# IntelLabs/bayesian-torch

Hardware: AMD Instinct MI355X
Metric: MC-samples/sec (Bayesian-ResNet18, 224^2, bs=64) (higher is better)
Workload: dtype bf16

## Files before the change

### bayesian_torch_amd/csrc/btx_contract.h

```cpp
#pragma once
#include <hip/hip_runtime.h>
#include <stdint.h>
#include "btx_rng.h"
#include "btx_plan.h"

typedef __attribute__((ext_vector_type(8))) __bf16 bf16x8;
typedef __attribute__((ext_vector_type(4))) __bf16 bf16x4;
typedef __attribute__((ext_vector_type(4))) float f32x4;
typedef __attribute__((ext_vector_type(8))) float f32x8;
typedef __attribute__((ext_vector_type(16))) float f32x16;
typedef __attribute__((ext_vector_type(4))) uint32_t u32x4;
typedef __attribute__((ext_vector_type(2))) uint32_t u32x2;

namespace btx {

constexpr int NTHREADS = 512;
constexpr int ACTS_OFF = 0;
constexpr int SIGN_OFF = NG * BM * 16;
constexpr int WMU_OFF = SIGN_OFF + NG * BM * 4;
constexpr int WDL_OFF = WMU_OFF + NG * BN * 16;
constexpr int STAGE_BYTES = WDL_OFF + NG * BN * 16;
constexpr int LDS_BYTES = 2 * STAGE_BYTES;

struct FastDiv {
  uint32_t m, sh;
};
static inline FastDiv make_fastdiv(uint32_t d) {
  FastDiv f;
  uint32_t l = 0;
  while ((1ull << l) < d) ++l;
  f.m = (uint32_t)((((1ull << l) - d) << 32) / d + 1);
  f.sh = (l < 1 ? l : 1) | ((l > 0 ? l - 1 : 0) << 8);
  return f;
}
__device__ __forceinline__ uint32_t fdiv(uint32_t x, const FastDiv& f) {
  const uint32_t t = __umulhi(x, f.m);
  return (t + ((x - t) >> (f.sh & 31u))) >> (f.sh >> 8);
}
static inline void sign_keys(const BtxRng* rng, uint32_t stream, uint32_t* ka, uint32_t* kb) {
  const BtxPhilox4 k = btx_philox4x32_10(0u, rng->sample_idx, rng->layer_id, stream, (uint32_t)rng->seed,
                                         (uint32_t)(rng->seed >> 32));
  *ka = k.x[0];
  *kb = k.x[1];
}
__device__ __forceinline__ void fdivmod(uint32_t x, const FastDiv& f, uint32_t d, uint32_t& q, uint32_t& r) {
  q = fdiv(x, f);
  r = x - q * d;
}

struct ContractParams {
  const void* x;
  const float* mu;
  const float* rho;
  const float* mu_b;
  const float* rho_b;
  void* out;
  float* partial;
  const float* eps_w;
  const float* eps_b;
  const int8_t* sign_in;
  const int8_t* sign_out;
  int NB, D, H, W, C, Cg;
  int Do, Ho, Wo, N, Ng;
  int KD, KH, KW;
  int sd, sh, sw, pd, ph, pw, dd, dh, dw;
  int M, K;
  int mtiles, ntiles, groups, ksplits, kper;
  int transposed;
  int pointwise;
  uint32_t seed_lo, seed_hi, sample, layer;
  const uint32_t* sample_ptr;
  uint32_t kin_a, kin_b, kout_a, kout_b;
  const float* ep_scale;
  const float* ep_shift;
  const void* ep_res;
  int ep_relu;
  int out_bf16;
  int sign_unaligned;
  uint32_t x_bytes, w_bytes;
  int pt_G, pt_R, pt_Rp, pt_Wp, pt_PP, pt_NI, pt_rtiles;
  FastDiv fd_Wo, fd_Ho, fd_Do, fd_ptWp, fd_ptRp, fd_ptR;
  FastDiv fd_inner, fd_ksplits, fd_ntiles, fd_Cg, fd_KW, fd_KH, fd_rtiles;
  FastDiv fd_mtiles;
  int swap_signs;
  int par_major, par_Mq, par_Mqp, par_Hh, par_Wh;
  FastDiv fd_par_Mqp, fd_par_Hh, fd_par_Wh;
  FastDiv fd_sd, fd_sh, fd_sw;
  int wg_order;
  int pt_nw, pt_astage, pt_lds;
  int pt_kg;
  int pt_lds_g;
  int pt_taps;
  int pt_wide;
  int sp_Hq, sp_Wq;
  int st_sbytes;
  void* wt;
  uint32_t wt_bytes, wt_delta_off;
  int wt_ready;
  int pt_tall, pt_P, pt_Wt, pt_ncs;
  FastDiv fd_P, fd_Wt, fd_ncs;
  int lanes, lane_nwg;
// ... 708 lines not shown
```

### bayesian_torch_amd/csrc/btx_contract_taps.h

```cpp
#pragma once
#include <type_traits>
#include "btx_contract.h"
#include "btx_contract_dma.h"
#include "btx_epilogue.h"
#include "btx_mma.h"

namespace btx {

__device__ __forceinline__ void dma16s(__amdgpu_buffer_rsrc_t rsrc, uint32_t voff, uint32_t soff,
                                       unsigned char* lds_wave_base) {
  __builtin_amdgcn_raw_ptr_buffer_load_lds(rsrc, (__attribute__((address_space(3))) void*)lds_wave_base, 16, voff, soff,
                                           0, 0);
}

template <int N>
__device__ __forceinline__ void end_stage() {
  asm volatile("s_waitcnt vmcnt(%0)\n\ts_waitcnt lgkmcnt(0)\n\ts_barrier" ::"n"(N) : "memory");
}

template <int I, int N, class F>
__device__ __forceinline__ void static_for(F&& f) {
  if constexpr (I < N) {
    f(std::integral_constant<int, I>{});
    static_for<I + 1, N>(f);
// ... 5 lines not shown
template <int T>
constexpr int tp_pieces(int t) {
  constexpr int PST = T - 3;
  constexpr int PPS = (TP_MAXNI + PST - 1) / PST;
  if (t < 0) t += T;
  if (t >= PST) return 0;
  int n = 0;
  for (int i = 0; i < PPS; ++i)
    if (t + PST * i < TP_MAXNI) ++n;
  return n;
}

template <int PREC, int KIND, int KH, int KW, int KG, bool WIDE = false>
__global__ __launch_bounds__(256 * KG, 2) void contract_taps_kernel(const ContractParams) {
  static_assert(!WIDE || (PREC == 1 && KG == 1 && KIND == 0), "wide tile: bf16 Reparameterization, one K-group");
  constexpr int K2 = (KIND == 1 || WIDE) ? 1 : 0;
  BTX_SECTION_PARAMS(p, logical);
  constexpr int NW = 4, NT = 256, MI = 2, T = KH * KW;
  static_assert(T >= 5 && T <= 32, "tap-unrolled kernel: 5..32 taps");
  constexpr int MAXNI = TP_MAXNI;
  constexpr int PST = T - 3;
  constexpr int WOPS = K2 ? 2 : 1;
  using ACT = typename std::conditional<PREC == 1, __bf16, float>::type;
  constexpr int G = (PREC == 1) ? 8 : 4;
  constexpr int BK = NG * G;
  constexpr int ESZ = (int)sizeof(ACT);
  extern __shared__ __attribute__((aligned(16))) unsigned char smem_all[];

  uint32_t smp = p.sample;
  if (p.sample_ptr) smp = sample_word_scalar(p.sample_ptr);

  const int tid = threadIdx.x & 255;
  const int lane = tid & 63;
  const int l31 = lane & 31;
  const int h = lane >> 5;
  const int wave_all = __builtin_amdgcn_readfirstlane((int)(threadIdx.x >> 6));
  const int wave = wave_all & 3;
  const int kg = (KG == 1) ? 0 : (wave_all >> 2);
  unsigned char* const smem = smem_all + kg * p.pt_lds_g;

  uint32_t u_mtile, u_rem, u_split, u_ntile, u_group, u_t;
  const uint32_t ntg = (uint32_t)(WIDE ? p.ntiles >> 1 : p.ntiles);
  if (p.wg_order) fdivmod((uint32_t)logical, p.fd_mtiles, (uint32_t)p.mtiles, u_rem, u_mtile);
  else fdivmod((uint32_t)logical, p.fd_inner, ntg * (uint32_t)(p.groups * p.ksplits), u_mtile, u_rem);
  fdivmod(u_rem, p.fd_ksplits, (uint32_t)p.ksplits, u_t, u_split);
  fdivmod(u_t, p.fd_ntiles, ntg, u_group, u_ntile);
  const int mtile = (int)u_mtile, split = (int)u_split, ntile = (int)u_ntile, group = (int)u_group;

  const bool tall = p.pt_tall != 0;
  uint32_t u_ig, u_rt;
  if (tall) fdivmod((uint32_t)mtile, p.fd_ncs, (uint32_t)p.pt_ncs, u_rt, u_ig);
  else fdivmod((uint32_t)mtile, p.fd_rtiles, (uint32_t)p.pt_rtiles, u_ig, u_rt);
  const int img0 = tall ? 0 : (int)u_ig * p.pt_G, row0 = (int)u_rt * p.pt_R, col0 = tall ? (int)u_ig * p.pt_Wt : 0;
  auto patch_src = [&](int q, bool& ok) __attribute__((always_inline)) -> uint32_t {
    uint32_t ut, upc, ugi, upr;
    fdivmod((uint32_t)q, p.fd_ptWp, (uint32_t)p.pt_Wp, ut, upc);
    int img, ih, iw;
    if (tall) {
      fdivmod((uint32_t)row0 + ut, p.fd_P, (uint32_t)p.pt_P, ugi, upr);
      img = (int)ugi; ih = (int)upr - p.ph; iw = col0 + (int)upc - p.pw;
      ok = (int)ut < p.pt_Rp;
    } else {
      fdivmod(ut, p.fd_ptRp, (uint32_t)p.pt_Rp, ugi, upr);
      img = img0 + (int)ugi; ih = row0 + (int)upr - p.ph; iw = (int)upc - p.pw;
      ok = true;
    }
    ok = ok && img < p.NB && (unsigned)ih < (unsigned)p.H && (unsigned)iw < (unsigned)p.W;
    return (uint32_t)((img * p.H + ih) * p.W + iw);
  };
  const int ncb_total = p.Cg / BK;
  const int cb_per = p.kper / BK;
  const int cb0 = split * cb_per + kg * (cb_per / KG);
  const int ncb = (KG == 1) ? min(ncb_total, cb0 + cb_per) - cb0 : cb_per / KG;
  const int a_stage = p.pt_astage, s_stage = p.pt_astage >> 4;
  const int PT_A_OFF = 0, PT_S_OFF = 2 * a_stage, PT_W_OFF = 2 * a_stage + 2 * s_stage;
  const int PT_X_OFF = PT_W_OFF + PT_WD * DW_STAGE;

  const __amdgpu_buffer_rsrc_t x_rsrc = __builtin_amdgcn_make_buffer_rsrc((void*)p.x, 0, p.x_bytes, 0x00020000);
  const __amdgpu_buffer_rsrc_t wt_rsrc = __builtin_amdgcn_make_buffer_rsrc((void*)p.wt, 0, p.wt_bytes, 0x00020000);

  const uint32_t w_voff = (uint32_t)lane * 16u + (uint32_t)wave * 1024u;
  const uint32_t w_sbase = (uint32_t)(group * p.ntiles + (WIDE ? 2 * ntile : ntile)) * (uint32_t)(p.K / G) * 1024u;
  const uint32_t w_second = WIDE ? (uint32_t)(p.K / G) * 1024u : p.wt_delta_off;
  const uint32_t CgG = (uint32_t)(p.Cg / G);
  const int w_lds = PT_W_OFF + wave * 1024;
  int wslot = 0;
  auto issue_w = [&](uint32_t tap, uint32_t cb, int slot) __attribute__((always_inline)) {
    const uint32_t soff = w_sbase + (tap * CgG + cb * (uint32_t)NG) * 1024u;
    unsigned char* ld = smem + w_lds + slot * DW_STAGE;
    dma16s(wt_rsrc, w_voff, soff, ld);
    if constexpr (K2) dma16s(wt_rsrc, w_voff, soff + w_second, ld + 4096);
  };
  if (ncb > 0) issue_w(0u, (uint32_t)cb0, 0);

  uint32_t sg_off[2];
  bool sg_ok[2];
  uint32_t* const pix_tab = (uint32_t*)(smem + PT_S_OFF + s_stage);
#pragma unroll
  for (int j = 0; j < 2; ++j) {
    const int q = tid + NT * j;
    sg_ok[j] = q < p.pt_PP;
    bool inside;
    const uint32_t ipix = patch_src(sg_ok[j] ? q : 0, inside);
    sg_off[j] = ipix * (uint32_t)p.C + (uint32_t)(group * p.Cg);
    if (q * 4 < s_stage) pix_tab[q] = (sg_ok[j] && inside) ? sg_off[j] : 0xffffffffu;
    if (p.sign_in)
      sg_ok[j] = sg_ok[j] && inside;
  }
  asm volatile("s_waitcnt lgkmcnt(0)\n\ts_barrier" ::: "memory");

  const int g_lane = (lane & 3) ^ ((lane >> 4) & 3);
  uint32_t pp_boff[MAXNI];
  uint32_t pmask = 0;
  uint32_t pp_e[MAXNI];
#pragma unroll
// ... 6 lines not shown
    const int q = 16 * (wave + NW * j) + (lane >> 2);
    uint32_t bo = DMA_OOB;
    if (j < p.pt_NI && q < p.pt_PP) {
      const uint32_t e = pp_e[j];
      if (e != 0xffffffffu) bo = (e + (uint32_t)(G * g_lane)) * (uint32_t)ESZ;
    }
    pp_boff[j] = bo;
    if (j < p.pt_NI && 16 * (wave + NW * j) < p.pt_PP) {
      pmask |= 1u << j;
      if (ncb > 0)
        dma16(x_rsrc, bo == DMA_OOB ? DMA_OOB : bo + (uint32_t)(cb0 * BK * ESZ), smem + PT_A_OFF + (wave + NW * j) * 1024);
    }
  }
  pmask = __builtin_amdgcn_readfirstlane(pmask);
  if (ncb > 0) {
    issue_w(1u, (uint32_t)cb0, 1);
    issue_w(2u, (uint32_t)cb0, 2);
  }

  RngLive rl = {smp, p.kin_a, p.kin_b, p.kout_a, p.kout_b};
  if (p.sample_ptr || p.lanes > 1) {
    rl.sample = __builtin_amdgcn_readfirstlane(smp);
    if constexpr (KIND == 1) {
      const uint32_t si = p.swap_signs ? 3u : 2u, so = p.swap_signs ? 2u : 3u;
      const BtxPhilox4 ki = btx_philox4x32_10(0u, rl.sample, p.layer, si, p.seed_lo, p.seed_hi);
      const BtxPhilox4 ko = btx_philox4x32_10(0u, rl.sample, p.layer, so, p.seed_lo, p.seed_hi);
      rl.kin_a = __builtin_amdgcn_readfirstlane(ki.x[0]); rl.kin_b = __builtin_amdgcn_readfirstlane(ki.x[1]);
      rl.kout_a = __builtin_amdgcn_readfirstlane(ko.x[0]); rl.kout_b = __builtin_amdgcn_readfirstlane(ko.x[1]);
    }
  }

  auto write_signs = [&](int slot, int cb) __attribute__((always_inline)) {
    if constexpr (KIND == 1) {
      unsigned char* ss = smem + PT_S_OFF + slot * s_stage;
#pragma unroll
      for (int j = 0; j < 2; ++j) {
        if (sg_ok[j]) {
          const uint32_t off = sg_off[j] + (uint32_t)(cb * BK);
          uint32_t w;
          if (p.sign_in) w = sign_word_explicit(p.sign_in, off, p.x_bytes / (uint32_t)ESZ);
          else w = btx_sign_word(off >> 5, rl.kin_a, rl.kin_b);
          if constexpr (G == 4) w <<= 8 * ((off >> 4) & 1);
          *(uint32_t*)(ss + (tid + NT * j) * 4) = w;
        }
      }
    }
  };

  int q0[MI];
#pragma unroll
  for (int mi = 0; mi < MI; ++mi) {
    const int pl = wave * 64 + mi * 32 + l31;
    uint32_t ut, uc, ugi, ur;
    if (tall) {
      fdivmod((uint32_t)pl, p.fd_Wt, (uint32_t)p.pt_Wt, ur, uc);
      q0[mi] = ((int)ur < p.pt_R) ? (int)ur * p.pt_Wp + (int)uc : 0;
    } else {
      fdivmod((uint32_t)pl, p.fd_Wo, (uint32_t)p.Wo, ut, uc);
      fdivmod(ut, p.fd_ptR, (uint32_t)p.pt_R, ugi, ur);
      const int c = (int)uc, r = (int)ur, gi = (int)ugi;
      const bool ok = (gi < p.pt_G) && (img0 + gi < p.NB) && (row0 + r < p.Ho);
      q0[mi] = ok ? (gi * p.pt_Rp + r) * p.pt_Wp + c : 0;
    }
  }
  const int row_step = p.dh * p.pt_Wp;

  constexpr bool ZI = (PREC == 1 && KG == 1);
  f32x16 accm[MI][2], accd[MI][2];
  auto clear_acc = [&](int a0) __attribute__((always_inline)) {
#pragma unroll
    for (int a = 0; a < MI; ++a)
#pragma unroll
      for (int b = 0; b < 2; ++b)
#pragma unroll
        for (int r = 0; r < 16; ++r)
          if (a >= a0) { accm[a][b][r] = 0.f; accd[a][b][r] = 0.f; }
  };
  if (!ZI || ncb <= 0) clear_acc(0);

  using Frag = StageFragT<MI>;
  auto load_frag = [&](Frag& f, int aslot, int toffv, int wsl, auto mia_tag) __attribute__((always_inline)) {
    constexpr int MIA = decltype(mia_tag)::value;
    const unsigned char* as = smem + PT_A_OFF + aslot * a_stage;
    const unsigned char* ss = smem + PT_S_OFF + aslot * s_stage;
    const unsigned char* ws = smem + PT_W_OFF + wsl * DW_STAGE;
    int q[MI];
#pragma unroll
    for (int mi = 0; mi < MI; ++mi) q[mi] = q0[mi] + toffv;
#pragma unroll
    for (int kk = 0; kk < NG / 2; ++kk) {
      const int row = 2 * kk + h;
#pragma unroll
      for (int mi = 0; mi < MIA; ++mi) f.a[kk][mi] = *(const u32x4*)(as + q[mi] * 64 + ((row ^ ((q[mi] >> 2) & 3)) * 16));
#pragma unroll
      for (int ni = 0; ni < 2; ++ni) f.wm[kk][ni] = *(const u32x4*)(ws + (row * BN + ni * 32 + l31) * 16);
    }
    if constexpr (KIND == 1) {
#pragma unroll
      for (int mi = 0; mi < MIA; ++mi) f.sw[mi] = *(const uint32_t*)(ss + q[mi] * 4);
    }
  };

  if (ncb > 0) {
    write_signs(0, cb0);
    asm volatile("s_waitcnt vmcnt(%0)\n\ts_waitcnt lgkmcnt(0)\n\ts_barrier" ::"n"(KG == 1 ? WOPS : 2 * WOPS) : "memory");
    Frag fa, fb;
    const int nvalid_px = tall ? p.pt_R * p.pt_Wt : min(p.pt_G, p.NB - img0) * min(p.pt_R, p.Ho - row0) * p.Wo;
    const bool mi1_dead = wave * 64 + 32 >= nvalid_px;
    auto kloop = [&](auto mia_tag) __attribute__((always_inline)) {
    constexpr int MIA = decltype(mia_tag)::value;
    if constexpr (KG == 1) load_frag(fa, 0, 0, 0, mia_tag);
    auto block = [&](auto par_tag, auto first_tag, int cbi, bool last) __attribute__((always_inline)) {
      constexpr int PAR = decltype(par_tag)::value;
      constexpr bool FIRST = decltype(first_tag)::value;
      static_for<0, T>([&](auto t_tag) __attribute__((always_inline)) {
        constexpr int t = decltype(t_tag)::value;
        constexpr int sp = (PAR * T + t) & 1;
        Frag& cur = (KG == 1 && sp) ? fb : fa;
        Frag& nxt = (KG == 1 && sp) ? fa : fb;
        asm volatile("" : "+v"(q0[0]), "+v"(q0[1]));
        constexpr int t3 = (t + 3) % T, c3 = (t + 3) / T;
        if constexpr (c3 == 0) {
          issue_w((uint32_t)t3, (uint32_t)(cb0 + cbi), (wslot + 3) & 3);
        } else {
          if (!last) issue_w((uint32_t)t3, (uint32_t)(cb0 + cbi + 1), (wslot + 3) & 3);
        }
        constexpr int KP = tp_pieces<T>(t);
        if constexpr (t < PST) {
          if (!last) {
            const uint32_t cboff = (uint32_t)((cb0 + cbi + 1) * BK * ESZ);
#pragma unroll
            for (int i = 0; i < KP; ++i) {
              const int j = t + PST * i;
              const uint32_t bo = pp_boff[j];
              unsigned char* dst = ((pmask >> j) & 1u) ? smem + PT_A_OFF + (PAR ^ 1) * a_stage + (wave + NW * j) * 1024
                                                        : smem + PT_X_OFF;
              dma16(x_rsrc, bo == DMA_OOB ? DMA_OOB : bo + cboff, dst);
            }
            if constexpr (t == 0) write_signs(PAR ^ 1, cb0 + cbi + 1);
          }
        }
        DeltaFrag df;
        if constexpr (KG == 1) {
          load_delta<K2>(df, smem + PT_W_OFF + wslot * DW_STAGE, l31, h);
          constexpr int t1 = (t + 1) % T, c1 = (t + 1) / T;
          load_frag(nxt, PAR ^ c1, (t1 / KW) * row_step + (t1 % KW) * p.dw, (wslot + 1) & 3, mia_tag);
          if constexpr (FIRST && t == 0) stage_mma<PREC, K2, MI, MIA, true, KIND == 1>(cur, df, accm, accd, l31, h);
          else stage_mma<PREC, K2, MI, MIA, false, KIND == 1>(cur, df, accm, accd, l31, h);
          if (!last) end_stage<WOPS + KP>();
          else end_stage<(c3 == 0) ? WOPS : 0>();
        } else {
          load_delta<KIND>(df, smem + PT_W_OFF + wslot * DW_STAGE, l31, h);
          load_frag(cur, PAR, (t / KW) * row_step + (t % KW) * p.dw, wslot, mia_tag);
          __builtin_amdgcn_sched_barrier(0);
          asm volatile("s_barrier" ::: "memory");
          __builtin_amdgcn_sched_barrier(0);
          stage_mma<PREC, KIND, MI, MIA>(cur, df, accm, accd, l31, h);
          __builtin_amdgcn_sched_barrier(0);
          if (!last) {
            end_stage<2 * WOPS + KP + tp_pieces<T>(t - 1) + tp_pieces<T>(t - 2)>();
          } else {
            constexpr int a_ = (t + 3 < T) ? 1 : 0, b_ = (t == 0) ? 1 : ((t + 2 < T) ? 1 : 0);
            end_stage<WOPS * (a_ + b_)>();
          }
        }
        wslot = (wslot + 1) & 3;
      });
    };
    if (KG == 2 && kg == 1) asm volatile("s_barrier" ::: "memory");
    using P0 = std::integral_constant<int, 0>;
    using P1 = std::integral_constant<int, 1>;
    if constexpr (ZI) {
      if constexpr (MIA < MI) clear_acc(MIA);
      block(P0{}, std::true_type{}, 0, ncb == 1);
      int cbi = 1;
      for (; cbi + 2 <= ncb; cbi += 2) {
        block(P1{}, std::false_type{}, cbi, false);
        block(P0{}, std::false_type{}, cbi + 1, cbi + 2 == ncb);
      }
      if (cbi < ncb) block(P1{}, std::false_type{}, cbi, true);
    } else {
      int cbi = 0;
      for (; cbi + 2 <= ncb; cbi += 2) {
        block(P0{}, std::false_type{}, cbi, false);
        block(P1{}, std::false_type{}, cbi + 1, cbi + 2 == ncb);
      }
      if (cbi < ncb) block(P0{}, std::false_type{}, cbi, true);
    }
    if (KG == 2 && kg == 0) asm volatile("s_barrier" ::: "memory");
    };
    if (mi1_dead) kloop(std::integral_constant<int, 1>{});
    else kloop(std::integral_constant<int, 2>{});
  }

  {
    BTX_SECTION_PARAMS(pe, logical2);
    const int nimg = min(pe.pt_G, pe.NB - img0), nrow = min(pe.pt_R, pe.Ho - row0);
    const int nvalid = nimg * nrow * pe.Wo;
    const uint32_t m0 = (uint32_t)(img0 * pe.Ho + row0) * (uint32_t)pe.Wo;
    const PixTall pmt = {pe, row0, col0};
    if constexpr (KG == 1) {
      if constexpr (WIDE) {
        float* const ba0 = (float*)(smem + NW * PT_EP_WAVE);
        float* const ba1 = ba0 + 4 * BN;
        {
          const bool has_bias = (split == 0) && (pe.mu_b != nullptr);
          const bool has_aff = (pe.ksplits == 1) && ((pe.ep_scale != nullptr) || (pe.ep_shift != nullptr));
          if (has_bias || has_aff) {
            if (tid < 64) ep_fill_constants<0>(pe, rl, ba0, tid, 2 * ntile, group, has_bias, has_aff);
            else if (tid < 128) ep_fill_constants<0>(pe, rl, ba1, tid - 64, 2 * ntile + 1, group, has_bias, has_aff);
          }
          __syncthreads();
        }
        if (tall) {
          staged_epilogue_pm<0, NW, PixTall>(pe, rl, accm, accm, smem, tid, wave, lane, 2 * ntile, group, split, pmt, -1, true, ba0);
          staged_epilogue_pm<0, NW, PixTall>(pe, rl, accd, accd, smem, tid, wave, lane, 2 * ntile + 1, group, split, pmt, -1, true, ba1);
        } else {
          staged_epilogue<0, NW>(pe, rl, accm, accm, smem, tid, wave, lane, 2 * ntile, group, split, m0, nvalid, -1, true, ba0);
          staged_epilogue<0, NW>(pe, rl, accd, accd, smem, tid, wave, lane, 2 * ntile + 1, group, split, m0, nvalid, -1, true, ba1);
        }
      } else
      if (tall) staged_epilogue_pm<KIND, NW, PixTall>(pe, rl, accm, accd, smem, tid, wave, lane, ntile, group, split, pmt);
      else staged_epilogue<KIND, NW>(pe, rl, accm, accd, smem, tid, wave, lane, ntile, group, split, m0, nvalid);
    } else {
      float* ba_lds = (float*)(smem_all + 131072);
      const bool to_partial = pe.ksplits > 1;
      const bool has_bias = (split == 0) && (pe.mu_b != nullptr);
      const bool has_aff = !to_partial && ((pe.ep_scale != nullptr) || (pe.ep_shift != nullptr));
      if (kg == 1) {
#pragma unroll
        for (int mi = 0; mi < MI; ++mi)
#pragma unroll
          for (int ni = 0; ni < 2; ++ni)
#pragma unroll
            for (int c = 0; c < 4; ++c) {
              const int i = (mi * 2 + ni) * 4 + c;
              *(f32x4*)(smem_all + (i * 256 + tid) * 16) =
                  (f32x4){accm[mi][ni][4 * c], accm[mi][ni][4 * c + 1], accm[mi][ni][4 * c + 2], accm[mi][ni][4 * c + 3]};
              if constexpr (KIND == 1)
                *(f32x4*)(smem_all + ((16 + i) * 256 + tid) * 16) =
                    (f32x4){accd[mi][ni][4 * c], accd[mi][ni][4 * c + 1], accd[mi][ni][4 * c + 2], accd[mi][ni][4 * c + 3]};
            }
      } else if (has_bias || has_aff) {
        ep_fill_constants<KIND>(pe, rl, ba_lds, tid, ntile, group, has_bias, has_aff);
      }
      __syncthreads();
      if (kg == 0) {
#pragma unroll
        for (int mi = 0; mi < MI; ++mi)
#pragma unroll
          for (int ni = 0; ni < 2; ++ni)
#pragma unroll
            for (int c = 0; c < 4; ++c) {
              const int i = (mi * 2 + ni) * 4 + c;
              const f32x4 v = *(const f32x4*)(smem_all + (i * 256 + tid) * 16);
#pragma unroll
              for (int r = 0; r < 4; ++r) accm[mi][ni][4 * c + r] += v[r];
              if constexpr (KIND == 1) {
                const f32x4 w = *(const f32x4*)(smem_all + ((16 + i) * 256 + tid) * 16);
#pragma unroll
                for (int r = 0; r < 4; ++r) accd[mi][ni][4 * c + r] += w[r];
              }
            }
      }
      __syncthreads();
      if (kg == 0) {
        if (tall) staged_epilogue_pm<KIND, NW, PixTall>(pe, rl, accm, accd, smem_all, tid, wave, lane, ntile, group, split, pmt, -1,
                                                        true, ba_lds);
        else staged_epilogue<KIND, NW>(pe, rl, accm, accd, smem_all, tid, wave, lane, ntile, group, split, m0, nvalid, -1, true,
                                       ba_lds);
      }
    }
  }
}

}
```

### bayesian_torch_amd/csrc/btx_epilogue.h

```cpp
#pragma once
#include <type_traits>
#include "btx_contract.h"

namespace btx {

template <int I, int N, class F>
__device__ __forceinline__ void static_for_ep(F&& f) {
  if constexpr (I < N) {
    f(std::integral_constant<int, I>{});
    static_for_ep<I + 1, N>(f);
  }
}

struct EpRaw {
  float mu, rho, eps, sc, sh;
};
__device__ __forceinline__ EpRaw ep_load_constants(const ContractParams& p, int t, int ntile, int group, bool has_bias,
                                                   bool has_aff) {
  EpRaw r = {0.f, 0.f, 0.f, 1.f, 0.f};
  if (t < BN) {
    const int col = ntile * BN + t;
    const int gcol = group * p.Ng + (col < p.Ng ? col : 0);
    if (has_bias && col < p.Ng) {
      r.mu = p.mu_b[gcol];
// ... 19 lines not shown
      else { bm = r.mu; bdl = sb_ * eb; }
    }
    ba_lds[t] = bm;
    ba_lds[BN + t] = bdl;
    ba_lds[2 * BN + t] = r.sc;
    ba_lds[3 * BN + t] = r.sh;
  }
}
template <int KIND>
__device__ __forceinline__ void ep_fill_constants(const ContractParams& p, const RngLive& rl, float* ba_lds, int t,
                                                  int ntile, int group, bool has_bias, bool has_aff) {
  const EpRaw r = ep_load_constants(p, t, ntile, group, has_bias, has_aff);
  ep_store_constants<KIND>(p, rl, r, ba_lds, t, ntile, group, has_bias);
}

struct PixContig {
  uint32_t m0;
  int nvalid;
  __device__ __forceinline__ uint32_t operator()(int pl, bool& ok) const { ok = pl < nvalid; return m0 + (uint32_t)pl; }
  __device__ __forceinline__ uint32_t first() const { return m0; }
  struct Walk {
    uint32_t g; int pl, nvalid;
    __device__ __forceinline__ uint32_t get(bool& ok) const { ok = pl < nvalid; return g; }
    __device__ __forceinline__ void step8() { g += 8u; pl += 8; }
  };
  __device__ __forceinline__ Walk walk(int pl) const { return Walk{m0 + (uint32_t)pl, pl, nvalid}; }
};
__device__ __forceinline__ uint32_t par_major_pixel(const ContractParams& p, uint32_t L) {
  uint32_t cls, q, t, b, nb, a;
  fdivmod(L, p.fd_par_Mqp, (uint32_t)p.par_Mqp, cls, q);
  fdivmod(q, p.fd_par_Wh, (uint32_t)p.par_Wh, t, b);
  fdivmod(t, p.fd_par_Hh, (uint32_t)p.par_Hh, nb, a);
  return (nb * (uint32_t)p.Ho + 2u * a + (cls >> 1)) * (uint32_t)p.Wo + 2u * b + (cls & 1u);
}
struct PixParity {
  const ContractParams& p;
  uint32_t m0;
  int nvalid;
  __device__ __forceinline__ uint32_t operator()(int pl, bool& ok) const {
    ok = pl < nvalid;
    return ok ? par_major_pixel(p, m0 + (uint32_t)pl) : 0u;
  }
  __device__ __forceinline__ uint32_t first() const { return 0u; }
  struct Walk {
    const ContractParams& p;
    uint32_t L; int pl, nvalid;
    __device__ __forceinline__ uint32_t get(bool& ok) const { ok = pl < nvalid; return ok ? par_major_pixel(p, L) : 0u; }
    __device__ __forceinline__ void step8() { L += 8u; pl += 8; }
  };
  __device__ __forceinline__ Walk walk(int pl) const { return Walk{p, m0 + (uint32_t)pl, pl, nvalid}; }
};
struct PixTall {
  const ContractParams& p;
  int row0, col0;
  __device__ __forceinline__ uint32_t operator()(int pl, bool& ok) const {
    uint32_t r, c, img, oh;
    fdivmod((uint32_t)pl, p.fd_Wt, (uint32_t)p.pt_Wt, r, c);
    fdivmod((uint32_t)row0 + r, p.fd_P, (uint32_t)p.pt_P, img, oh);
    const int ow = col0 + (int)c;
    ok = (int)r < p.pt_R && (int)oh < p.Ho && (int)img < p.NB && ow < p.Wo;
    return ok ? ((img * (uint32_t)p.Ho + oh) * (uint32_t)p.Wo + (uint32_t)ow) : 0u;
  }
  __device__ __forceinline__ uint32_t first() const { return 0u; }
  struct Walk {
    const ContractParams& p;
    int r, c, oh, img, col0;
    __device__ __forceinline__ uint32_t get(bool& ok) const {
      const int ow = col0 + c;
      ok = r < p.pt_R && oh < p.Ho && img < p.NB && ow < p.Wo;
      return ok ? (uint32_t)((img * p.Ho + oh) * p.Wo + ow) : 0u;
    }
    __device__ __forceinline__ void step8() {
      c += 8;
#pragma unroll
      for (int i = 0; i < 2; ++i)
        if (c >= p.pt_Wt) { c -= p.pt_Wt; ++r; if (++oh >= p.pt_P) { oh -= p.pt_P; ++img; } }
    }
  };
  __device__ __forceinline__ Walk walk(int pl) const {
    uint32_t r, c, img, oh;
    fdivmod((uint32_t)pl, p.fd_Wt, (uint32_t)p.pt_Wt, r, c);
    fdivmod((uint32_t)row0 + r, p.fd_P, (uint32_t)p.pt_P, img, oh);
    return Walk{p, (int)r, (int)c, (int)oh, (int)img, col0};
  }
};

struct EpNoHook {
  __device__ __forceinline__ void operator()() const {}
};
template <int KIND, int NW, class PM = PixContig, bool RES_PRE = false, class HOOK = EpNoHook>
__device__ __forceinline__ void staged_epilogue_pm(const ContractParams& p, const RngLive& rl, const f32x16 (&accm)[2][2],
                                                   const f32x16 (&accd)[2][2], unsigned char* smem, int tid, int wave,
                                                   int lane, int ntile, int group, int split, const PM& pm,
                                                   int pwave = -1, bool first = true,
                                                   float* ba_ext = nullptr, const HOOK& hook = HOOK{},
                                                   const uint32_t* wsh_ext = nullptr) {
  if (pwave < 0) pwave = wave;
  constexpr int EP_ROW = PT_EP_ROW;
  constexpr int EP_WAVE = PT_EP_WAVE;
  const int l31 = lane & 31, h = lane >> 5;
  const bool to_partial = p.ksplits > 1;
  const bool has_bias = (split == 0) && (p.mu_b != nullptr);
  const bool has_aff = !to_partial && ((p.ep_scale != nullptr) || (p.ep_shift != nullptr));
  const bool has_ba = has_bias || has_aff;
  float* ba_lds = ba_ext ? ba_ext : (float*)(smem + NW * EP_WAVE);
  if (has_ba && first && !ba_ext) {
    ep_fill_constants<KIND>(p, rl, ba_lds, tid, ntile, group, has_bias, has_aff);
    __syncthreads();
  }
  unsigned char* ep = smem + wave * EP_WAVE;

  constexpr bool BUFIO = RES_PRE && std::is_same<PM, PixContig>::value;
  u32x4 rpre[8];
  auto io_off = [&](int lane_) __attribute__((always_inline)) -> uint32_t {
    return ((pm.first() + (uint32_t)(pwave * 64 + (lane_ >> 3))) * (uint32_t)p.N + (uint32_t)(group * p.Ng + ntile * BN + (lane_ & 7) * 8)) * 2u;
  };
  const uint32_t io_step = 8u * (uint32_t)p.N * 2u, io_bytes = (uint32_t)p.M * (uint32_t)p.N * 2u;
  if constexpr (RES_PRE) {
    const bool all_vec = ((p.N & 7) == 0) && (((group * p.Ng) & 7) == 0) && (ntile * BN + BN <= p.Ng);
    if (all_vec && !to_partial && p.ep_res != nullptr && p.out_bf16 && p.ep_relu != 2) {
      if constexpr (BUFIO) {
        const __amdgpu_buffer_rsrc_t res_rsrc = __builtin_amdgcn_make_buffer_rsrc((void*)p.ep_res, 0, io_bytes, 0x00020000);
        const uint32_t io_voff = io_off(lane);
#pragma unroll
        for (int i = 0; i < 8; ++i) rpre[i] = __builtin_amdgcn_raw_buffer_load_b128(res_rsrc, io_voff, io_step * (uint32_t)i, 0);
      } else {
        const uint32_t cbase = (uint32_t)(group * p.Ng + ntile * BN + (lane & 7) * 8);
        auto wk = pm.walk(pwave * 64 + (lane >> 3));
#pragma unroll
        for (int i = 0; i < 8; ++i) {
          bool ok;
          const uint32_t gp = wk.get(ok);
          wk.step8();
          rpre[i] = *(const u32x4*)((const __bf16*)p.ep_res + (ok ? gp * (uint32_t)p.N + cbase : cbase + pm.first() * (uint32_t)p.N));
        }
      }
// ... 258 lines not shown
```

### bayesian_torch_amd/csrc/btx_plan.cpp

```cpp
#include <string.h>
#include "btx_plan.h"

namespace btx {

static inline long long plan_lanes(uint32_t flags) {
  const long long n = (flags >> BTX_FLAG_LANES_SHIFT) & 0xffu;
  return n > 1 ? n : 1;
}

static inline bool throughput_plan(uint32_t flags) { return (flags & BTX_FLAG_CONCURRENT) || plan_lanes(flags) > 1; }

static int split_k(long long base1, int units, int unit_cost, int max_split, bool full_splits, bool throughput, bool short_exit) {
  int ks = 1;
  long long best = -1;
  for (int c = 1; c <= max_split; ++c) {
    if (full_splits && units % c) continue;
    const int per = (units + c - 1) / c;
    const long long rounds = (base1 * c + SLOTS - 1) / SLOTS;
    const long long cost = rounds * (per * unit_cost + 4) + (c > 1 ? 1 : 0);
    if (best < 0 || cost < best) { best = cost; ks = c; }
    if (throughput && (base1 * c >= 64 || (short_exit && base1 * c >= 16 && per <= 16))) { ks = c; break; }
  }
  return ks;
}
// ... 7 lines not shown
  const long long M = (long long)g->NB * pl->Do * pl->Ho * pl->Wo;
  const long long K = (long long)g->KD * g->KH * g->KW * pl->Cg;
  if (M > 0x7fffffffLL || K > 0x7fffffffLL) return BTX_E_UNSUPPORTED;
  pl->M = (int)M;
  pl->K = (int)K;
  const int bk = NG * (prec == BTX_PREC_BF16 ? 8 : 4);
  pl->mtiles = (pl->M + bm - 1) / bm;
  pl->ntiles = (pl->Ng + BN - 1) / BN;
  const long long base1 = (long long)pl->mtiles * pl->ntiles * g->groups;
  const int stages = (pl->K + bk - 1) / bk;
  const int max_ks = stages / 4 > 1 ? (stages / 4 < 32 ? stages / 4 : 32) : 1;
  const int ks = split_k(base1, stages, 1, max_ks, false, throughput_plan(flags), true);
  int per_stages = (stages + ks - 1) / ks;
  pl->kper = per_stages * bk;
  pl->ksplits = (pl->K + pl->kper - 1) / pl->kper;
  const long long nwg = base1 * pl->ksplits;
  if (nwg > 0x7fffffffLL) return BTX_E_UNSUPPORTED;
  pl->nwg = (int)nwg;
  return 0;
}

static bool dma_shape_ok(const BtxGeom* g, int act_dtype, int prec, const Plan& pl) {
  if ((prec == BTX_PREC_BF16) != (act_dtype == BTX_ACT_BF16)) return false;
  const int bk = NG * (prec == BTX_PREC_BF16 ? 8 : 4);
  if (pl.Cg % bk) return false;
  const long long in_elems = (long long)g->NB * g->D * g->H * g->W * g->C;
  const long long esz = (act_dtype == BTX_ACT_BF16) ? 2 : 4;
  if (in_elems * esz >= 0xfff00000LL || (long long)pl.M * g->N >= 0x7fffffffLL ||
      (long long)g->N * pl.K * 4 >= 0xfff00000LL)
    return false;
  return true;
}

static double tall_tile(const BtxGeom* g, const Plan& pl, int tp, int ppcap, PatchPlan* pt) {
  const int halo_r = (g->KH - 1) * g->dh, halo_c = (g->KW - 1) * g->dw;
  if (g->ph > halo_r) return 0.0;
  const int P = (g->H + g->ph > pl.Ho) ? g->H + g->ph : pl.Ho;
  const long long rows_total = (long long)(g->NB - 1) * P + pl.Ho;
  double best = 0.0;
  for (int ncs = 1; ncs <= 8; ++ncs) {
    const int Wt = (pl.Wo + ncs - 1) / ncs;
    if (Wt > tp || Wt < 4 || (ncs > 1 && Wt < 8)) continue;
    int R = tp / Wt;
    if (R > rows_total) R = (int)rows_total;
    while (R >= 1 && (R + halo_r) * (Wt + halo_c) > ppcap) --R;
    if (R < 1) continue;
    const long long rtiles = (rows_total + R - 1) / R;
    const double eff = (double)pl.M / ((double)rtiles * ncs * tp);
    if (eff > best * 1.01) {
      best = eff;
      pt->tall = 1; pt->P = P; pt->Wt = Wt; pt->ncs = ncs;
      pt->G = 1; pt->R = R; pt->Rp = R + halo_r; pt->Wp = Wt + halo_c; pt->PP = pt->Rp * pt->Wp;
      pt->rtiles = (int)rtiles;
    }
  }
  return best;
}
static bool patch_tile(const BtxGeom* g, const Plan& pl, int tp, int ppcap, PatchPlan* pt) {
  const int Ho = pl.Ho, Wo = pl.Wo;
  const int Wp = Wo + (g->KW - 1) * g->dw, halo_r = (g->KH - 1) * g->dh;
  if (Wo > tp || Wp * (1 + halo_r) > ppcap) return false;
  int G = 1, R;
  if (Ho * Wo <= tp / 2 || (Ho * Wo <= tp && (Ho + halo_r) * Wp <= ppcap)) {
    R = Ho;
    const int Rp = R + halo_r;
    if (Rp * Wp > ppcap) return false;
    G = tp / (Ho * Wo);
    if (G > ppcap / (Rp * Wp)) G = ppcap / (Rp * Wp);
    if (G > g->NB) G = g->NB;
    if (G < 1) return false;
  } else {
    int rmax = tp / Wo;
    const int rfit = ppcap / Wp - halo_r;
    if (rfit < rmax) rmax = rfit;
    if (rmax > Ho) rmax = Ho;
    if (rmax < 1) return false;
    const int nrt = (Ho + rmax - 1) / rmax;
    R = (Ho + nrt - 1) / nrt;
    auto mfma_tiles = [&](int r) {
      long long n = 0;
      for (int row = 0; row < Ho; row += r) n += ((long long)((Ho - row < r) ? Ho - row : r) * Wo + 31) / 32;
      return n;
    };
    if (rmax > R && (Ho % rmax == 0 || 2 * (Ho % rmax) >= rmax) && mfma_tiles(rmax) < mfma_tiles(R)) R = rmax;
  }
  pt->G = G; pt->R = R; pt->Rp = R + halo_r; pt->Wp = Wp; pt->PP = G * pt->Rp * Wp;
  pt->rtiles = (Ho + R - 1) / R;
  return pt->PP <= ppcap && G * R * Wo <= tp;
}


static bool patch_base_ok(const BtxGeom* g, int act_dtype, int prec, uint32_t flags, Plan* pl, PatchPlan* pt) {
  if (flags & (BTX_FLAG_TRANSPOSED | BTX_FLAG_ROWFUSE)) return false;
  pt->wide = 0;
  if (make_plan(g, prec, flags, DBM, pl)) return false;
  if (!dma_shape_ok(g, act_dtype, prec, *pl)) return false;
  return g->D == 1 && g->KD == 1 && pl->Do == 1;
}
static bool patch_lds(PatchPlan* pt, int slots, int wd, int max_ni) {
  const int pieces = (pt->PP + 15) / 16;
  pt->NI = (pieces + pt->nw - 1) / pt->nw;
  if (pt->NI > max_ni) return false;
  pt->astage = pieces * 1024;
  int lds = slots * pt->astage + slots * (pt->astage / 16) + wd * 8192 + 1024;
  const int ep = pt->nw * PT_EP_WAVE + 1024;
  if (lds < ep) lds = ep;
  if (lds > (pt->nw == 4 ? 81920 : 163840)) return false;
  pt->lds = lds;
  pt->lds_g = (lds + 15) & ~15;
  return true;
}
static void wide_tile(const BtxGeom* g, int kind, int act_dtype, int prec, uint32_t flags, const Plan& pl, PatchPlan* pt) {
  if (kind == BTX_KIND_REPARAM && prec == BTX_PREC_BF16 && act_dtype == BTX_ACT_BF16 && (pl.Ng % 128) == 0 &&
      (long long)pl.mtiles * (pl.ntiles / 2) * g->groups * plan_lanes(flags) >= SLOTS) {
    pt->wide = 1;
    if (pt->lds < pt->nw * PT_EP_WAVE + 2048) {
      pt->lds = pt->nw * PT_EP_WAVE + 2048;
      pt->lds_g = (pt->lds + 15) & ~15;
    }
  }
}
static long long patch_base1(const BtxGeom* g, const Plan& pl, const PatchPlan& pt) {
  return (long long)pl.mtiles * (pt.wide ? pl.ntiles / 2 : pl.ntiles) * g->groups;
}
static bool patch_split_k(const BtxGeom* g, int prec, uint32_t flags, int T, Plan* pl, const PatchPlan& pt) {
  const int bk = NG * (prec == BTX_PREC_BF16 ? 8 : 4);
  const int units = pl->Cg / bk / pt.kg;
  const long long base1 = patch_base1(g, *pl, pt);
  const long long base1n = throughput_plan(flags) ? (long long)pl->mtiles * pl->ntiles * g->groups : base1;
  int max_ks = 1;
  while (max_ks < units && max_ks < 32 && (units + max_ks) / (max_ks + 1) * T >= 4) ++max_ks;
  const int ks = split_k(base1n, units, T, max_ks, pt.kg == 2, throughput_plan(flags), false);
  const int per = (units + ks - 1) / ks;
  pl->kper = per * pt.kg * bk;
  pl->ksplits = (units + per - 1) / per;
  const long long nwg = base1 * pl->ksplits;
  if (nwg > 0x7fffffffLL) return false;
  pl->nwg = (int)nwg;
  return true;
}

static bool make_patch_plan(const BtxGeom* g, int act_dtype, int prec, uint32_t flags, Plan* pl, PatchPlan* pt, int kind = -1) {
  if (!patch_base_ok(g, act_dtype, prec, flags, pl, pt) || g->sh != 1 || g->sw != 1) return false;
  const int T = g->KH * g->KW;
  if (T < 2 || T > 64) return false;
  pt->tall = 0; pt->P = 1; pt->Wt = 1; pt->ncs = 1;
  if (patch_tile(g, *pl, 256, 352, pt)) pt->nw = 4;
  else if (patch_tile(g, *pl, 512, 960, pt)) pt->nw = 8;
  else return false;
  if (pt->nw == 4 && g->KH == 3 && g->KW == 3) {
    const long long mt_old = (long long)((g->NB + pt->G - 1) / pt->G) * pt->rtiles;
    const double eff_old = (double)pl->M / ((double)mt_old * 256.0);
    PatchPlan tp = *pt;
    const double eff_tall = tall_tile(g, *pl, 256, 352, &tp);
    if (eff_tall > eff_old * TALL_MIN_GAIN) *pt = tp;
  }
  if (!patch_lds(pt, 2, PT_WD, PT_MAXNI)) return false;
  pl->mtiles = pt->tall ? pt->rtiles * pt->ncs : ((g->NB + pt->G - 1) / pt->G) * pt->rtiles;
  pt->taps = (pt->nw == 4 && pt->NI <= 6 && g->KH == 3 && g->KW == 3) ? 33 : 0;
  if (pt->taps == 33) wide_tile(g, kind, act_dtype, prec, flags, *pl, pt);
  const int ncb = pl->Cg / (NG * (prec == BTX_PREC_BF16 ? 8 : 4));
  pt->kg = (pt->taps && !throughput_plan(flags) && patch_base1(g, *pl, *pt) * plan_lanes(flags) <= 256 && ncb >= 2 && (ncb % 2) == 0 &&
            2 * pt->lds_g <= 163840) ? 2 : 1;
  if (!patch_split_k(g, prec, flags, T, pl, *pt)) return false;
  if (pt->kg == 2) pt->lds = 2 * pt->lds_g;
  return true;
}

static bool make_patch2_plan(const BtxGeom* g, int act_dtype, int prec, uint32_t flags, Plan* pl, PatchPlan* pt, int kind = -1) {
  if (!patch_base_ok(g, act_dtype, prec, flags, pl, pt)) return false;
  if (g->KH != 3 || g->KW != 3 || g->sh != 2 || g->sw != 2 || g->ph != 1 || g->pw != 1 || g->dh != 1 || g->dw != 1) return false;
  BtxGeom gp = *g;
  gp.KH = 2; gp.KW = 2;
  if (!patch_tile(&gp, *pl, 256, 272, pt)) return false;
  pt->nw = 4;
  pt->tall = 0; pt->P = 1; pt->Wt = 1; pt->ncs = 1;
  if (!patch_lds(pt, 3, 3, 5)) return false;
  pl->mtiles = ((g->NB + pt->G - 1) / pt->G) * pt->rtiles;
  wide_tile(g, kind, act_dtype, prec, flags, *pl, pt);
  pt->taps = 332;
  pt->kg = 1;
  return patch_split_k(g, prec, flags, 9, pl, *pt);
}

static bool make_stem_plan(const BtxGeom* g, int act_dtype, int prec, const Plan& pl, StemPlan* st) {
  if (g->D != 1 || g->KD != 1 || pl.Do != 1 || g->groups != 1) return false;
  const int esz = (act_dtype == BTX_ACT_BF16) ? 2 : 4;
  const int bk = NG * (prec == BTX_PREC_BF16 ? 8 : 4);
  if ((g->KW * g->C) % bk || pl.K % bk) return false;
  const long long rowB = (long long)g->W * g->C * esz;
  for (int nw = 4; nw <= 8; nw += 4) {
    const int tp = 64 * nw;
    if (pl.Wo > tp) continue;
    int R = tp / pl.Wo;
    if (R > pl.Ho) R = pl.Ho;
    const long long cap = (nw == 4 ? 81920 : 163840) - PT_WD * 8192;
    for (; R >= 1; --R) {
      const long long Rp = (long long)(R - 1) * g->sh + g->KH;
      const long long pb = Rp * rowB;
      const long long astage = (pb + 1023) / 1024 * 1024;
      const long long sbytes = ((pb / esz + 31) / 32 + 3) * 4;
      const long long sb16 = (sbytes + 15) / 16 * 16;
      if (astage + sb16 > cap) continue;
      long long lds = astage + sb16 + PT_WD * 8192;
      const long long ep = (long long)nw * PT_EP_WAVE + 1024;
      if (lds < ep) lds = ep;
      st->R = R; st->Rp = (int)Rp; st->rtiles = (pl.Ho + R - 1) / R; st->nw = nw; st->astage = (int)astage;
      st->sbytes = (int)sb16; st->lds = (int)lds; st->patch_bytes = (int)pb;
      const long long nwg = (long long)g->NB * st->rtiles * pl.ntiles;
      if (nwg > 0x7fffffffLL) return false;
      st->nwg = (int)nwg;
      return true;
    }
  }
  return false;
}

// ... 271 lines not shown
```

### bayesian_torch_amd/csrc/btx_plan.h

```cpp
#pragma once
#include <stddef.h>
#include <stdint.h>
#include "../../include/btx.h"

namespace btx {

constexpr int BM = 256;
constexpr int BN = 64;
constexpr int NG = 4;
constexpr int DBM = 512;

constexpr int PT_WD = 4;
constexpr int PT_EP_ROW = 272;
constexpr int PT_EP_WAVE = 64 * PT_EP_ROW;
constexpr int PT_MAXNI = 8;

constexpr long long SLOTS = 256;
constexpr double TALL_MIN_GAIN = 1.15;
constexpr int GEMM8_MIN_K = 128;
constexpr double WG_MAJOR_MIB = 3.0;

struct Plan {
  int Do, Ho, Wo, Cg, Ng, M, K, mtiles, ntiles, ksplits, kper, nwg;
};

struct PatchPlan {
  int G, R, Rp, Wp, PP, NI, rtiles, nw, astage, lds;
  int taps, kg, lds_g;
  int wide;
  int tall, P, Wt, ncs;
};

struct StemPlan {
  int R, Rp, rtiles, nw, astage, sbytes, lds, patch_bytes, nwg;
};

struct StemPoolPlan {
  int PB, bands, Rp, astage, sbytes, lds, patch_bytes, nwg, Hq, Wq;
};

struct FwdSel {
  int family;
  Plan pl;
  int par_major;
  int par_mqp, g8_pairs, out_bf16;
  StemPlan stp;
  StemPoolPlan spp;
  PatchPlan pt;
  size_t need, wt_off, wt_one, wt_all;
};
static inline bool uses_tiles(int family) { return family >= BTX_FAMILY_DMA; }

int select_fwd(int kind, const BtxGeom* g, int act_dtype, int prec, uint32_t flags, bool unaligned, const BtxNoise* noise,
               const BtxEpilogue* ep, FwdSel* s);

int make_plan(const BtxGeom* g, int prec, uint32_t flags, int bm, Plan* pl);
size_t plan_ws(const Plan& pl, const BtxGeom* g, int lanes = 1);
size_t patch_wt_bytes(const Plan& pl, const BtxGeom* g, int kind, int prec, size_t* one, int lanes = 1);

}
```

Measured before the change: 1920.

## Add dense cross-image row tiling for 3x3 patch conv to cut padded tiles

Adds a new 'dense' tiling mode (tall=2) for 3x3 patch convolutions that treats all images' output rows as one continuous sequence, so a tile can span image boundaries. The planner picks it only when it needs no more MFMA work and no more workgroups than the legacy tiling. The aim is to reduce wasted MFMA work and workgroup count on small spatial layers such as 7x7 and 14x14, where per-image tiles leave lanes idle. In exchange, patch index math, the epilogue pixel mapping and the LDS halo rows become more complex, and each patch carries extra padding rows between images.

```diff
diff --git a/bayesian_torch_amd/csrc/btx_contract.h b/bayesian_torch_amd/csrc/btx_contract.h
--- a/bayesian_torch_amd/csrc/btx_contract.h
+++ b/bayesian_torch_amd/csrc/btx_contract.h
@@ -47,6 +47,12 @@
   q = fdiv(x, f);
   r = x - q * d;
 }
+
+struct FdDiv {
+  FastDiv f;
+  uint32_t d;
+  __device__ __forceinline__ void operator()(uint32_t x, uint32_t& q, uint32_t& r) const { fdivmod(x, f, d, q, r); }
+};
 
 struct ContractParams {
   const void* x;
diff --git a/bayesian_torch_amd/csrc/btx_contract_taps.h b/bayesian_torch_amd/csrc/btx_contract_taps.h
--- a/bayesian_torch_amd/csrc/btx_contract_taps.h
+++ b/bayesian_torch_amd/csrc/btx_contract_taps.h
@@ -81,15 +81,16 @@
   if (tall) fdivmod((uint32_t)mtile, p.fd_ncs, (uint32_t)p.pt_ncs, u_rt, u_ig);
   else fdivmod((uint32_t)mtile, p.fd_rtiles, (uint32_t)p.pt_rtiles, u_ig, u_rt);
   const int img0 = tall ? 0 : (int)u_ig * p.pt_G, row0 = (int)u_rt * p.pt_R, col0 = tall ? (int)u_ig * p.pt_Wt : 0;
+  const int patch_row0 = (p.pt_tall == 2) ? dense_ov(row0, p.pt_P, FdDiv{p.fd_Ho, (uint32_t)p.Ho}) : row0;
   auto patch_src = [&](int q, bool& ok) __attribute__((always_inline)) -> uint32_t {
     uint32_t ut, upc, ugi, upr;
-    fdivmod((uint32_t)q, p.fd_ptWp, (uint32_t)p.pt_Wp, ut, upc);
     int img, ih, iw;
     if (tall) {
-      fdivmod((uint32_t)row0 + ut, p.fd_P, (uint32_t)p.pt_P, ugi, upr);
-      img = (int)ugi; ih = (int)upr - p.ph; iw = col0 + (int)upc - p.pw;
-      ok = (int)ut < p.pt_Rp;
+      int prow;
+      strip_patch_src(q, patch_row0, col0, p.ph, p.pw, FdDiv{p.fd_ptWp, (uint32_t)p.pt_Wp}, FdDiv{p.fd_P, (uint32_t)p.pt_P}, prow, img, ih, iw);
+      ok = prow < p.pt_Rp;
     } else {
+      fdivmod((uint32_t)q, p.fd_ptWp, (uint32_t)p.pt_Wp, ut, upc);
       fdivmod(ut, p.fd_ptRp, (uint32_t)p.pt_Rp, ugi, upr);
       img = img0 + (int)ugi; ih = row0 + (int)upr - p.ph; iw = (int)upc - p.pw;
       ok = true;
@@ -202,7 +203,12 @@
   for (int mi = 0; mi < MI; ++mi) {
     const int pl = wave * 64 + mi * 32 + l31;
     uint32_t ut, uc, ugi, ur;
-    if (tall) {
+    if (p.pt_tall == 2) {
+      int rr, c;
+      dense_slot(pl, row0, FdDiv{p.fd_Wt, (uint32_t)p.pt_Wt}, rr, c);
+      q0[mi] = (rr - row0 < min(p.pt_R, p.NB * p.Ho - row0))
+                   ? dense_patch_pixel(rr, c, patch_row0, p.pt_P, p.pt_Wp, FdDiv{p.fd_Ho, (uint32_t)p.Ho}) : 0;
+    } else if (tall) {
       fdivmod((uint32_t)pl, p.fd_Wt, (uint32_t)p.pt_Wt, ur, uc);
       q0[mi] = ((int)ur < p.pt_R) ? (int)ur * p.pt_Wp + (int)uc : 0;
     } else {
@@ -255,7 +261,9 @@
     write_signs(0, cb0);
     asm volatile("s_waitcnt vmcnt(%0)\n\ts_waitcnt lgkmcnt(0)\n\ts_barrier" ::"n"(KG == 1 ? WOPS : 2 * WOPS) : "memory");
     Frag fa, fb;
-    const int nvalid_px = tall ? p.pt_R * p.pt_Wt : min(p.pt_G, p.NB - img0) * min(p.pt_R, p.Ho - row0) * p.Wo;
+    const int nvalid_px = (p.pt_tall == 2) ? min(p.pt_R, p.NB * p.Ho - row0) * p.pt_Wt
+                          : tall           ? p.pt_R * p.pt_Wt
+                                           : min(p.pt_G, p.NB - img0) * min(p.pt_R, p.Ho - row0) * p.Wo;
     const bool mi1_dead = wave * 64 + 32 >= nvalid_px;
     auto kloop = [&](auto mia_tag) __attribute__((always_inline)) {
     constexpr int MIA = decltype(mia_tag)::value;
@@ -346,9 +354,10 @@
   {
     BTX_SECTION_PARAMS(pe, logical2);
     const int nimg = min(pe.pt_G, pe.NB - img0), nrow = min(pe.pt_R, pe.Ho - row0);
-    const int nvalid = nimg * nrow * pe.Wo;
-    const uint32_t m0 = (uint32_t)(img0 * pe.Ho + row0) * (uint32_t)pe.Wo;
-    const PixTall pmt = {pe, row0, col0};
+    const bool dense = pe.pt_tall == 2, strips = tall && !(dense && pe.pt_ncs == 1);
+    const int nvalid = dense ? min(pe.pt_R, pe.NB * pe.Ho - row0) * pe.Wo : nimg * nrow * pe.Wo;
+    const uint32_t m0 = (uint32_t)(dense ? row0 : img0 * pe.Ho + row0) * (uint32_t)pe.Wo;
+    const PixTall pmt = {pe, row0, col0, dense ? pe.Ho : pe.pt_P, dense ? pe.fd_Ho : pe.fd_P};
     if constexpr (KG == 1) {
       if constexpr (WIDE) {
         float* const ba0 = (float*)(smem + NW * PT_EP_WAVE);
@@ -362,7 +371,7 @@
           }
           __syncthreads();
         }
-        if (tall) {
+        if (strips) {
           staged_epilogue_pm<0, NW, PixTall>(pe, rl, accm, accm, smem, tid, wave, lane, 2 * ntile, group, split, pmt, -1, true, ba0);
           staged_epilogue_pm<0, NW, PixTall>(pe, rl, accd, accd, smem, tid, wave, lane, 2 * ntile + 1, group, split, pmt, -1, true, ba1);
         } else {
@@ -370,7 +379,7 @@
           staged_epilogue<0, NW>(pe, rl, accd, accd, smem, tid, wave, lane, 2 * ntile + 1, group, split, m0, nvalid, -1, true, ba1);
         }
       } else
-      if (tall) staged_epilogue_pm<KIND, NW, PixTall>(pe, rl, accm, accd, smem, tid, wave, lane, ntile, group, split, pmt);
+      if (strips) staged_epilogue_pm<KIND, NW, PixTall>(pe, rl, accm, accd, smem, tid, wave, lane, ntile, group, split, pmt);
       else staged_epilogue<KIND, NW>(pe, rl, accm, accd, smem, tid, wave, lane, ntile, group, split, m0, nvalid);
     } else {
       float* ba_lds = (float*)(smem_all + 131072);
@@ -415,7 +424,7 @@
       }
       __syncthreads();
       if (kg == 0) {
-        if (tall) staged_epilogue_pm<KIND, NW, PixTall>(pe, rl, accm, accd, smem_all, tid, wave, lane, ntile, group, split, pmt, -1,
+        if (strips) staged_epilogue_pm<KIND, NW, PixTall>(pe, rl, accm, accd, smem_all, tid, wave, lane, ntile, group, split, pmt, -1,
                                                         true, ba_lds);
         else staged_epilogue<KIND, NW>(pe, rl, accm, accd, smem_all, tid, wave, lane, ntile, group, split, m0, nvalid, -1, true,
                                        ba_lds);
diff --git a/bayesian_torch_amd/csrc/btx_epilogue.h b/bayesian_torch_amd/csrc/btx_epilogue.h
--- a/bayesian_torch_amd/csrc/btx_epilogue.h
+++ b/bayesian_torch_amd/csrc/btx_epilogue.h
@@ -95,11 +95,12 @@
 };
 struct PixTall {
   const ContractParams& p;
-  int row0, col0;
+  int row0, col0, P;
+  FastDiv fdP;
   __device__ __forceinline__ uint32_t operator()(int pl, bool& ok) const {
     uint32_t r, c, img, oh;
     fdivmod((uint32_t)pl, p.fd_Wt, (uint32_t)p.pt_Wt, r, c);
-    fdivmod((uint32_t)row0 + r, p.fd_P, (uint32_t)p.pt_P, img, oh);
+    fdivmod((uint32_t)row0 + r, fdP, (uint32_t)P, img, oh);
     const int ow = col0 + (int)c;
     ok = (int)r < p.pt_R && (int)oh < p.Ho && (int)img < p.NB && ow < p.Wo;
     return ok ? ((img * (uint32_t)p.Ho + oh) * (uint32_t)p.Wo + (uint32_t)ow) : 0u;
@@ -107,7 +108,7 @@
   __device__ __forceinline__ uint32_t first() const { return 0u; }
   struct Walk {
     const ContractParams& p;
-    int r, c, oh, img, col0;
+    int r, c, oh, img, col0, P;
     __device__ __forceinline__ uint32_t get(bool& ok) const {
       const int ow = col0 + c;
       ok = r < p.pt_R && oh < p.Ho && img < p.NB && ow < p.Wo;
@@ -117,14 +118,14 @@
       c += 8;
 #pragma unroll
       for (int i = 0; i < 2; ++i)
-        if (c >= p.pt_Wt) { c -= p.pt_Wt; ++r; if (++oh >= p.pt_P) { oh -= p.pt_P; ++img; } }
+        if (c >= p.pt_Wt) { c -= p.pt_Wt; ++r; if (++oh >= P) { oh -= P; ++img; } }
     }
   };
   __device__ __forceinline__ Walk walk(int pl) const {
     uint32_t r, c, img, oh;
     fdivmod((uint32_t)pl, p.fd_Wt, (uint32_t)p.pt_Wt, r, c);
-    fdivmod((uint32_t)row0 + r, p.fd_P, (uint32_t)p.pt_P, img, oh);
-    return Walk{p, (int)r, (int)c, (int)oh, (int)img, col0};
+    fdivmod((uint32_t)row0 + r, fdP, (uint32_t)P, img, oh);
+    return Walk{p, (int)r, (int)c, (int)oh, (int)img, col0, P};
   }
 };
 
diff --git a/bayesian_torch_amd/csrc/btx_plan.cpp b/bayesian_torch_amd/csrc/btx_plan.cpp
--- a/bayesian_torch_amd/csrc/btx_plan.cpp
+++ b/bayesian_torch_amd/csrc/btx_plan.cpp
@@ -83,6 +83,42 @@
       pt->tall = 1; pt->P = P; pt->Wt = Wt; pt->ncs = ncs;
       pt->G = 1; pt->R = R; pt->Rp = R + halo_r; pt->Wp = Wt + halo_c; pt->PP = pt->Rp * pt->Wp;
       pt->rtiles = (int)rtiles;
+    }
+  }
+  return best;
+}
+static long long legacy_mfma(const BtxGeom* g, const Plan& pl, const PatchPlan& pt) {
+  if (pt.tall) return (long long)pt.rtiles * pt.ncs * tile_mfma(pt.R * pt.Wt);
+  auto group = [&](int nimg) {
+    long long n = 0;
+    for (int row0 = 0; row0 < pl.Ho; row0 += pt.R) n += tile_mfma(nimg * (pl.Ho - row0 < pt.R ? pl.Ho - row0 : pt.R) * pl.Wo);
+    return n;
+  };
+  return (long long)(g->NB / pt.G) * group(pt.G) + (g->NB % pt.G ? group(g->NB % pt.G) : 0);
+}
+long long dense_tile(const BtxGeom* g, const Plan& pl, int tp, int ppcap, long long max_mfma, long long max_wg, PatchPlan* pt) {
+  const int halo_r = (g->KH - 1) * g->dh, halo_c = (g->KW - 1) * g->dw;
+  if (g->ph > halo_r) return 0;
+  const int P = (g->H + g->ph > pl.Ho) ? g->H + g->ph : pl.Ho;
+  const long long rows_total = (long long)g->NB * pl.Ho;
+  long long best = 0, best_wg = 0;
+  for (int ncs = 1; ncs <= 8; ++ncs) {
+    const int Wt = (pl.Wo + ncs - 1) / ncs;
+    if (Wt > tp || Wt < 4 || (ncs > 1 && Wt < 8)) continue;
+    for (int R = (tp / Wt < rows_total) ? tp / Wt : (int)rows_total; R >= 1; --R) {
+      const int Rp = dense_rp_max(R, pl.Ho, P, halo_r);
+      if ((long long)Rp * (Wt + halo_c) > ppcap) continue;
+      const long long rtiles = (rows_total + R - 1) / R;
+      const int tail = (int)(rows_total - (rtiles - 1) * R);
+      const long long mfma = ((rtiles - 1) * tile_mfma(R * Wt) + tile_mfma(tail * Wt)) * ncs, wg = rtiles * ncs;
+      if (mfma > max_mfma || wg > max_wg || (mfma == max_mfma && wg == max_wg)) continue;
+      if (best == 0 || wg < best_wg || (wg == best_wg && mfma < best)) {
+        best = mfma; best_wg = wg;
+        pt->tall = 2; pt->P = P; pt->Wt = Wt; pt->ncs = ncs;
+        pt->G = 1; pt->R = R; pt->Rp = Rp; pt->Wp = Wt + halo_c; pt->PP = Rp * pt->Wp;
+        pt->rtiles = (int)rtiles;
+        pt->mfma = mfma;
+      }
     }
   }
   return best;
@@ -141,14 +177,17 @@
   pt->lds_g = (lds + 15) & ~15;
   return true;
 }
+static void wide_lds(PatchPlan* pt) {
+  if (pt->lds < pt->nw * PT_EP_WAVE + 2048) {
+    pt->lds = pt->nw * PT_EP_WAVE + 2048;
+    pt->lds_g = (pt->lds + 15) & ~15;
+  }
+}
 static void wide_tile(const BtxGeom* g, int kind, int act_dtype, int prec, uint32_t flags, const Plan& pl, PatchPlan* pt) {
   if (kind == BTX_KIND_REPARAM && prec == BTX_PREC_BF16 && act_dtype == BTX_ACT_BF16 && (pl.Ng % 128) == 0 &&
       (long long)pl.mtiles * (pl.ntiles / 2) * g->groups * plan_lanes(flags) >= SLOTS) {
     pt->wide = 1;
-    if (pt->lds < pt->nw * PT_EP_WAVE + 2048) {
-      pt->lds = pt->nw * PT_EP_WAVE + 2048;
-      pt->lds_g = (pt->lds + 15) & ~15;
-    }
+    wide_lds(pt);
   }
 }
 static long long patch_base1(const BtxGeom* g, const Plan& pl, const PatchPlan& pt) {
@@ -189,11 +228,26 @@
   if (!patch_lds(pt, 2, PT_WD, PT_MAXNI)) return false;
   pl->mtiles = pt->tall ? pt->rtiles * pt->ncs : ((g->NB + pt->G - 1) / pt->G) * pt->rtiles;
   pt->taps = (pt->nw == 4 && pt->NI <= 6 && g->KH == 3 && g->KW == 3) ? 33 : 0;
+  PatchPlan dn = *pt;
+  bool dense = false;
+  if (pt->taps == 33) {
+    pt->mfma = legacy_mfma(g, *pl, *pt);
+    dense = dense_tile(g, *pl, 256, 352, pt->mfma, pl->mtiles, &dn) > 0 && patch_lds(&dn, 2, PT_WD, 6);
+  }
   if (pt->taps == 33) wide_tile(g, kind, act_dtype, prec, flags, *pl, pt);
   const int ncb = pl->Cg / (NG * (prec == BTX_PREC_BF16 ? 8 : 4));
   pt->kg = (pt->taps && !throughput_plan(flags) && patch_base1(g, *pl, *pt) * plan_lanes(flags) <= 256 && ncb >= 2 && (ncb % 2) == 0 &&
             2 * pt->lds_g <= 163840) ? 2 : 1;
   if (!patch_split_k(g, prec, flags, T, pl, *pt)) return false;
+  if (dense) {
+    dn.wide = pt->wide; dn.kg = pt->kg;
+    if (dn.wide) wide_lds(&dn);
+    *pt = dn;
+    pl->mtiles = pt->rtiles * pt->ncs;
+    const long long nwg = patch_base1(g, *pl, *pt) * pl->ksplits;
+    if (nwg > 0x7fffffffLL) return false;
+    pl->nwg = (int)nwg;
+  }
   if (pt->kg == 2) pt->lds = 2 * pt->lds_g;
   return true;
 }
diff --git a/bayesian_torch_amd/csrc/btx_plan.h b/bayesian_torch_amd/csrc/btx_plan.h
--- a/bayesian_torch_amd/csrc/btx_plan.h
+++ b/bayesian_torch_amd/csrc/btx_plan.h
@@ -29,7 +29,49 @@
   int taps, kg, lds_g;
   int wide;
   int tall, P, Wt, ncs;
+  long long mfma;
 };
+
+#if defined(__HIPCC__)
+#define BTX_PLAN_HD __host__ __device__
+#else
+#define BTX_PLAN_HD
+#endif
+struct PlainDiv {
+  uint32_t d;
+  BTX_PLAN_HD void operator()(uint32_t x, uint32_t& q, uint32_t& r) const { q = x / d; r = x - q * d; }
+};
+template <class DIV>
+BTX_PLAN_HD inline int dense_ov(int rr, int P, const DIV& div_Ho) {
+  uint32_t img, oh;
+  div_Ho((uint32_t)rr, img, oh);
+  return (int)img * P + (int)oh;
+}
+template <class DIV>
+BTX_PLAN_HD inline void dense_slot(int pl, int rr0, const DIV& div_Wt, int& rr, int& c) {
+  uint32_t r, cc;
+  div_Wt((uint32_t)pl, r, cc);
+  rr = rr0 + (int)r;
+  c = (int)cc;
+}
+template <class DIV>
+BTX_PLAN_HD inline int dense_patch_pixel(int rr, int c, int ov0, int P, int Wp, const DIV& div_Ho) {
+  return (dense_ov(rr, P, div_Ho) - ov0) * Wp + c;
+}
+template <class DW, class DP>
+BTX_PLAN_HD inline void strip_patch_src(int q, int v0, int col0, int ph, int pw, const DW& div_Wp, const DP& div_P, int& ut,
+                                        int& img, int& ih, int& iw) {
+  uint32_t t, pc, gi, pr;
+  div_Wp((uint32_t)q, t, pc);
+  div_P((uint32_t)v0 + t, gi, pr);
+  ut = (int)t; img = (int)gi; ih = (int)pr - ph; iw = col0 + (int)pc - pw;
+}
+BTX_PLAN_HD inline int dense_rp_max(int R, int Ho, int P, int halo_r) { return R + (R - 1 + Ho - 1) / Ho * (P - Ho) + halo_r; }
+BTX_PLAN_HD inline int tile_mfma(int nvalid) {
+  int n = 0;
+  for (int w = 0; w < 4; ++w) n += (w * 64 + 32 >= nvalid) ? 1 : 2;
+  return n;
+}
 
 struct StemPlan {
   int R, Rp, rtiles, nw, astage, sbytes, lds, patch_bytes, nwg;
@@ -55,6 +97,7 @@
                const BtxEpilogue* ep, FwdSel* s);
 
 int make_plan(const BtxGeom* g, int prec, uint32_t flags, int bm, Plan* pl);
+long long dense_tile(const BtxGeom* g, const Plan& pl, int tp, int ppcap, long long max_mfma, long long max_wg, PatchPlan* pt);
 size_t plan_ws(const Plan& pl, const BtxGeom* g, int lanes = 1);
 size_t patch_wt_bytes(const Plan& pl, const BtxGeom* g, int kind, int prec, size_t* one, int lanes = 1);
 
```

Result: faster. 1989, median of 6 (+3.6%).
